# wangjie212/ManiSDP-matlab

Measured on AMD Instinct MI355X. Metric: tCG Hess-vec prods/sec (n,p), G81 MaxCut, higher is better.
Workload: dtype f64; 1 GPU; Gset G81 MaxCut, ManiSDP_onlyunitdiag RTR call, n=20000, p=32; n=20000, p=32, nnz_C=92644, TR_maxiter=40, TR_maxinner=100, parallelism=rows1

## Files before the change

include/manisdp_hip.h:

```cpp
#ifndef MANISDP_HIP_H
#define MANISDP_HIP_H

#include <stdint.h>

#ifdef __cplusplus
extern "C" {
#endif

#define MSDP_OK              0
#define MSDP_EINVAL         -1
#define MSDP_EHIP           -2
#define MSDP_ENOMEM         -3
#define MSDP_ESTATE         -4
#define MSDP_ECOMM          -5
#define MSDP_EUNSUPPORTED   -6

typedef struct msdp_handle_s* msdp_handle;

#define MSDP_KIND_ONLYUNITDIAG 1
#define MSDP_KIND_UNITDIAG     2
#define MSDP_KIND_UNITTRACE    3
#define MSDP_KIND_GENERIC      4
#define MSDP_KIND_MULTIBLOCK   5
#define MSDP_KIND_DUAL_UNITDIAG 6
// ... 137 lines not shown
int msdp_local_rows(msdp_handle h, int64_t* row0, int64_t* row1);


int msdp_al_primal(msdp_handle h, double* obj, double* Ax);
int msdp_al_dual(msdp_handle h, const double* y, double* z);
int msdp_escape_eigs_dual(msdp_handle h, int32_t k, double tol, int32_t maxit,
                          double* lam_min, double* V, double* lam_max, int32_t* iters);
int msdp_get_dual_slack(msdp_handle h, double* S);
int msdp_get_dual_slack_block(msdp_handle h, int64_t row0, int64_t nb, double* S);
int msdp_block_eigs(msdp_handle h, int32_t nb, const int64_t* row0, const int64_t* nblk, int32_t k, int32_t method, double* w, double* V);
#define MSDP_BLOCK_EIGS_LARGE_MAXN 1024
int msdp_block_eigs_large(msdp_handle h, int32_t nb, const int64_t* row0, const int64_t* nblk, int32_t k, double* w, double* V);
int msdp_block_eigs_large_info(msdp_handle h, int32_t* launches, int32_t* workgroups);
#define MSDP_BLOCK_RESHAPE_MAXP 64
int msdp_block_reshape(msdp_handle h, int32_t nb, const int64_t* row0, const int64_t* nblk, const int32_t* p_in,
                       const double* w, const double* V, int32_t k, double theta, int32_t strict, int32_t delta,
                       double alpha, int32_t min_facsize, int32_t mode,
                       int32_t* p_out, int32_t* r_out, int32_t* nne_out, double* U);

int msdp_set_option(msdp_handle h, const char* name, int32_t value);

int msdp_tcg_path(msdp_handle h, int32_t* path);
int msdp_debug_persist_form(msdp_handle h, int32_t* form);


int msdp_bench_hessvec(msdp_handle h, int32_t reps, double* avg_ms,
                       double* algo_bytes, double* algo_flops);
int msdp_bench_kernel(msdp_handle h, int32_t which, int32_t reps, double* avg_ms);
int msdp_bench_tcg_trip(msdp_handle h, int32_t reps, double* avg_ms);

const char* msdp_last_error(void);
const char* msdp_version(void);

#ifdef __cplusplus
}
#endif
#endif
```

manisdp-matlab_amd/_lib.py:

```python
from __future__ import annotations

import ctypes as C
import os

import numpy as np

_HERE = os.path.dirname(os.path.abspath(__file__))
LIB_PATH = os.path.join(_HERE, "lib", "libmanisdp_hip.so")

KIND_ONLYUNITDIAG, KIND_UNITDIAG, KIND_UNITTRACE, KIND_GENERIC, KIND_MULTIBLOCK, KIND_DUAL_UNITDIAG, KIND_DUAL = 1, 2, 3, 4, 5, 6, 7
KIND_DUAL_MULTIBLOCK = 8


class RtrOpts(C.Structure):
    _fields_ = [("maxiter", C.c_int32), ("maxinner", C.c_int32), ("mininner", C.c_int32),
                ("reserved0", C.c_int32), ("tolgradnorm", C.c_double), ("kappa", C.c_double),
                ("theta", C.c_double), ("rho_prime", C.c_double), ("rho_regularization", C.c_double),
                ("Delta_bar", C.c_double), ("Delta0", C.c_double)]


class RtrStats(C.Structure):
    _fields_ = [("cost", C.c_double), ("gradnorm", C.c_double), ("Delta", C.c_double),
                ("seconds", C.c_double), ("iters", C.c_int32), ("hessvecs", C.c_int32),
                ("accepted", C.c_int32), ("rejected", C.c_int32), ("cost_evals", C.c_int32),
# ... 73 lines not shown
    "msdp_comm_init_local": (C.c_int, [C.c_void_p, C.c_int32, C.c_int32, C.c_int32]),
    "msdp_comm_init_ipc": (C.c_int, [C.c_void_p, C.c_int32, C.c_int32, C.c_char_p]),
    "msdp_get_point_all": (C.c_int, [C.c_void_p, _dp]),
    "msdp_get_z_all": (C.c_int, [C.c_void_p, _dp]),
    "msdp_factor_gram": (C.c_int, [C.c_void_p, _dp]),
    "msdp_factor_rotate": (C.c_int, [C.c_void_p, C.c_int32, _dp]),
    "msdp_factor_append": (C.c_int, [C.c_void_p, C.c_int32, _dp, C.c_double, C.c_int32]),
    "msdp_create_dual_unitdiag": (C.c_int, [C.c_int64, C.c_int64, _i64p, _i64p, _dp, _dp, _dp, _dp, C.c_int32, _i64p, _i64p, _dp,
                                            _dp, C.c_int32, C.POINTER(C.c_void_p)]),
    "msdp_create_dual": (C.c_int, [C.c_int64, C.c_int64, _i64p, _i64p, _dp, _dp, _dp, _dp, C.c_int32, _i64p, _i64p, _dp,
                                   _dp, C.c_int32, C.POINTER(C.c_void_p)]),
    "msdp_create_dual_multiblock": (C.c_int, [C.c_int32, _i64p, C.c_int32, C.c_int64, _i64p, _i64p, _dp, _dp, _dp, _dp, C.c_int32,
                                              _i64p, _i64p, _dp, _dp, C.c_int32, C.POINTER(C.c_void_p)]),
    "msdp_dual_info": (C.c_int, [C.c_void_p, _P(C.c_int32)]),
    "msdp_dual_set_penalty": (C.c_int, [C.c_void_p, C.c_double, _dp]),
    "msdp_dual_outer_step": (C.c_int, [C.c_void_p, _dp, _dp, _dp]),
    "msdp_dual_get_y": (C.c_int, [C.c_void_p, _dp]),
    "msdp_comm_unique_id": (C.c_int, [C.c_void_p]),
    "msdp_comm_init": (C.c_int, [C.c_void_p, C.c_int32, C.c_int32, C.c_void_p]),
    "msdp_local_rows": (C.c_int, [C.c_void_p, _i64p, _i64p]),
    "msdp_debug_shard": (C.c_int, [C.c_void_p, C.c_int32, C.c_int32]),
    "msdp_tcg_path": (C.c_int, [C.c_void_p, _P(C.c_int32)]),
    "msdp_debug_persist_form": (C.c_int, [C.c_void_p, _P(C.c_int32)]),
    "msdp_point_snapshot": (C.c_int, [C.c_void_p]),
    "msdp_point_restore": (C.c_int, [C.c_void_p]),
    "msdp_al_primal": (C.c_int, [C.c_void_p, _dp, _dp]),
    "msdp_al_dual": (C.c_int, [C.c_void_p, _dp, _dp]),
    "msdp_escape_eigs_dual": (C.c_int, [C.c_void_p, C.c_int32, C.c_double, C.c_int32, _dp, _dp, _dp, _P(C.c_int32)]),
    "msdp_bench_hessvec": (C.c_int, [C.c_void_p, C.c_int32, _dp, _dp, _dp]),
    "msdp_bench_tcg_trip": (C.c_int, [C.c_void_p, C.c_int32, _dp]),
    "msdp_bench_kernel": (C.c_int, [C.c_void_p, C.c_int32, C.c_int32, _dp]),
    "msdp_last_error": (C.c_char_p, []),
    "msdp_version": (C.c_char_p, []),
}

_lib = None


def load():
    global _lib
    if _lib is not None:
        return _lib
    if not os.path.exists(LIB_PATH):
        raise MsdpError(f"{LIB_PATH} not found: run `python -c 'import __graft_entry__ as g; g.build()'` "
                        "(or `make -C manisdp-matlab_amd/csrc`). There is no CPU fallback.")
    lib = C.CDLL(LIB_PATH)
# ... 1 lines not shown
        fn = getattr(lib, name)
        fn.restype = res
        fn.argtypes = args
    _lib = lib
    import atexit
    atexit.register(lambda: lib.msdp_release_cache())
    return lib


def release_cache():
    _check(load().msdp_release_cache())


def pool_stats():
    a, b, c = C.c_int64(), C.c_int64(), C.c_int64()
    _check(load().msdp_debug_pool_stats(C.byref(a), C.byref(b), C.byref(c)))
    return a.value, b.value, c.value


def mem_info():
    a, b = C.c_int64(), C.c_int64()
    _check(load().msdp_debug_mem_info(C.byref(a), C.byref(b)))
    return a.value, b.value


def _check(rc):
    if rc != 0:
        err = MsdpError(f"libmanisdp_hip error {rc}: {load().msdp_last_error().decode()}")
        err.code = rc
        raise err


def _dptr(a):
    return a.ctypes.data_as(_dp)


def set_device(dev):
    _check(load().msdp_set_device(int(dev)))


def device_count():
    n = C.c_int32()
    _check(load().msdp_device_count(C.byref(n)))
    return n.value


# ... 502 lines not shown
```

manisdp-matlab_amd/csrc/msdp_api.hip:

```cpp
#include "msdp_common.h"
#include <algorithm>
#include <cmath>
#include <cstdarg>
#include <cstdio>
#include <cstdlib>
#include <cstring>

static thread_local char g_err[1024] = "";
void msdp_set_error(const char* fmt, ...) {
    va_list ap;
    va_start(ap, fmt);
    vsnprintf(g_err, sizeof(g_err), fmt, ap);
    va_end(ap);
}
extern "C" const char* msdp_last_error(void) { return g_err; }
extern "C" const char* msdp_version(void) { return "manisdp_hip 0.1.0 (gfx950)"; }

static bool boundary_colmajor(msdp_handle h) { return h->kind == MSDP_KIND_UNITTRACE || h->kind == MSDP_KIND_GENERIC || h->kind == MSDP_KIND_DUAL; }

static void choose_grid(msdp_handle h) {
    Dev& d = h->d;
    int half = d.ld / 2, lpr = 1;
    while (lpr < half && lpr < 64) lpr <<= 1;
    const int rows_per_step = MSDP_WAVES * (64 / lpr);
// ... 95 lines not shown
static int new_handle(int kind, int64_t n, msdp_handle* out) {
    if (!out) { msdp_set_error("out handle pointer is null"); return MSDP_EINVAL; }
    if (n <= 0 || n > 0x7fffffff) { msdp_set_error("matrix order n = %lld out of range", (long long)n); return MSDP_EINVAL; }
    int ndev = 0;
    if (hipGetDeviceCount(&ndev) != hipSuccess || ndev == 0) {
        msdp_set_error("no HIP device visible: libmanisdp_hip has no CPU fallback");
        return MSDP_EHIP;
    }
    msdp_handle h = new msdp_handle_s();
    h->kind = kind;
    h->d.n = (int)n;
    h->d.n_loc = (int)n;
    h->d.row0 = 0;
    h->d.manifold = (kind == MSDP_KIND_UNITTRACE) ? MANI_SPHERE : (kind == MSDP_KIND_GENERIC ? MANI_EUCLID : MANI_OBLIQUE);
    {
        auto on = [](const char* name) { const char* e = getenv(name); return e && atoi(e) != 0; };
        if (on("MSDP_NO_PERSIST")) h->tune.persist = 0;
        if (on("MSDP_NO_FUSED_RTR")) h->tune.fused_rtr = 0;
        if (on("MSDP_NO_PERSIST_PIPE")) h->tune.persist_pipe = 0;
        if (on("MSDP_NO_GRAPH")) h->tune.graph = 0;
        if (on("MSDP_TIMING")) h->tune.timing = 1;
        if (on("MSDP_ESC_DEBUG")) h->tune.esc_debug = 1;
        h->d.persist_ep = h->tune.persist_ep;
        if (const char* e = getenv("MSDP_AFFINE_ROUTE")) h->tune.affine_route = !strcmp(e, "gram") ? 2 : (!strcmp(e, "sddmm") ? 1 : 0);
    }
    hipError_t e = hipSuccess;
    if (!msdp_host_kit_take(h)) {
        e = hipStreamCreateWithFlags(&h->stream, hipStreamNonBlocking);
        if (e == hipSuccess) e = hipHostMalloc((void**)&h->h_ctl, sizeof(Ctl), hipHostMallocDefault);
        if (e == hipSuccess) e = hipHostMalloc((void**)&h->h_frame, 2 * sizeof(Frame), hipHostMallocDefault);
        if (e == hipSuccess) e = hipHostMalloc((void**)&h->h_flags, 64, hipHostMallocDefault);
        if (e == hipSuccess) e = hipHostMalloc((void**)&h->h_status, 64, hipHostMallocMapped);
    }
    if (e == hipSuccess) e = hipEventCreate(&h->ev0);
    if (e == hipSuccess) e = hipEventCreate(&h->ev1);
    if (e == hipSuccess) e = hipEventCreateWithFlags(&h->ev_flag[0], hipEventDisableTiming);
    if (e == hipSuccess) e = hipEventCreateWithFlags(&h->ev_flag[1], hipEventDisableTiming);
    if (e == hipSuccess) {
        *h->h_status = 0;
        void* dp = nullptr;
        e = hipHostGetDevicePointer(&dp, (void*)h->h_status, 0);
        h->d.status = (unsigned long long*)dp;
    }
    if (e != hipSuccess) {
        msdp_set_error("stream/event/pinned setup failed: %s", hipGetErrorString(e));
        delete h;
// ... 653 lines not shown
    if (!name) { msdp_set_error("set_option: null name"); return MSDP_EINVAL; }
    Tuning& t = h->tune;
    if (!strcmp(name, "persist")) t.persist = value != 0;
    else if (!strcmp(name, "fused_rtr")) t.fused_rtr = value != 0;
    else if (!strcmp(name, "graph")) { t.graph = value != 0; h->chunk_len = 0; }
    else if (!strcmp(name, "affine_route")) { if (value < 0 || value > 2) { msdp_set_error("affine_route: 0 auto, 1 sddmm, 2 gram"); return MSDP_EINVAL; } t.affine_route = value; h->chunk_len = 0; h->state_valid = false; }
    else if (!strcmp(name, "timing")) t.timing = value != 0;
    else if (!strcmp(name, "esc_debug")) t.esc_debug = value != 0;
    else if (!strcmp(name, "escape_deflate")) t.escape_deflate = value != 0;
    else if (!strcmp(name, "escape_warm")) t.escape_warm = value != 0;
    else if (!strcmp(name, "escape_start_y")) t.escape_start_y = value != 0;
    else if (!strcmp(name, "xpersist")) t.xpersist = value != 0;
    else if (!strcmp(name, "persist_refresh")) t.persist_refresh = value > 0 ? value : 0;
    else if (!strcmp(name, "xtail")) t.xtail = value ? 1 : 0;
    else if (!strcmp(name, "xr_twolevel")) t.xr_twolevel = value ? 1 : 0;
    else if (!strcmp(name, "window")) { t.window = value < 0 ? 0 : (value > 3 ? 3 : value); h->chunk_len = 0; }
    else if (!strcmp(name, "window_lds")) { t.window_lds = value < 16 ? 16 : (value > 144 ? 144 : value); h->chunk_len = 0; msdp_window_release(h); }
    else if (!strcmp(name, "persist_early")) t.persist_early = value > 0 ? value : 0;
    else if (!strcmp(name, "persist_pipe")) t.persist_pipe = value > 0 ? 1 : 0;
    else if (!strcmp(name, "pipe_refresh")) t.pipe_refresh = value > 0 ? (value < 2 ? 2 : value) : 0;
    else if (!strcmp(name, "pipe_local")) t.pipe_local = value > 0 ? 1 : 0;
    else if (!strcmp(name, "persist_goff")) t.persist_goff = value ? 1 : 0;
    else if (!strcmp(name, "persist_ep")) { t.persist_ep = value ? 1 : 0; h->d.persist_ep = t.persist_ep; h->persist_sig_fn = nullptr; }
    else if (!strcmp(name, "persist_slots")) { t.persist_slots = (value == 3 || value == 4) ? value : 0; h->d.persist_slots = t.persist_slots; }
    else if (!strcmp(name, "psync_backoff")) t.psync_backoff = value > 0 ? value : 0;
    else if (!strcmp(name, "psync8_backoff")) t.psync8_backoff = value > 0 ? (value > 255 ? 255 : value) : 0;
    else if (!strcmp(name, "affine_overlap")) { t.affine_overlap = value != 0; h->chunk_len = 0; }
    else if (!strcmp(name, "trip1")) { t.trip1 = value < 0 ? 0 : (value > 2 ? 2 : value); h->chunk_len = 0; }
    else if (!strcmp(name, "dense_sk")) t.dense_sk = value < 0 ? 0 : value;
    else if (!strcmp(name, "sweep_k")) { t.sweep_k = value < 1 ? 1 : value; choose_grid(h); h->chunk_len = 0; }
    else if (!strcmp(name, "sweep")) { t.sweep = value < 0 ? 0 : (value > 3 ? 3 : value); choose_grid(h); h->chunk_len = 0; }
    else if (!strcmp(name, "trip2")) { t.trip2 = value < 0 ? 0 : (value > 2 ? 2 : value); h->chunk_len = 0; }
    else if (!strcmp(name, "escape_method")) { if (value < 0 || value > 2) { msdp_set_error("escape_method: 0 auto, 1 lanczos, 2 block"); return MSDP_EINVAL; } t.escape_method = value; }
    else if (!strcmp(name, "be_width")) { if (value != 0 && value != 32 && value != 64 && value != 128) { msdp_set_error("be_width: 0, 32, 64 or 128"); return MSDP_EINVAL; } t.be_width = value; }
    else if (!strcmp(name, "be_degree")) t.be_degree = value > 0 ? value : 0;
    else if (!strcmp(name, "be_grid")) t.be_grid = value > 0 ? (value > MSDP_MAX_GRID ? MSDP_MAX_GRID : value) : 0;
    else if (!strcmp(name, "be_lpr")) { if (value != 0 && value != 8 && value != 16 && value != 32 && value != 64) { msdp_set_error("be_lpr: 0, 8, 16, 32 or 64"); return MSDP_EINVAL; } t.be_lpr = value; }
    else if (!strcmp(name, "lanczos_onesync")) t.lanczos_onesync = value != 0;
    else if (!strcmp(name, "lanczos_qglobal")) t.lanczos_qglobal = value != 0;
    else if (!strcmp(name, "block_skip")) t.block_skip = value != 0;
    else if (!strcmp(name, "halo_exchange")) { t.halo_exchange = value != 0; h->state_valid = false; }
    else if (!strcmp(name, "dense_pack")) { t.dense_pack = value != 0; h->chunk_len = 0; }
    else if (!strcmp(name, "affine_fuse")) { t.affine_fuse = value != 0; h->chunk_len = 0; h->state_valid = false; }
    else if (!strcmp(name, "affine_side")) { t.affine_side = value != 0; h->chunk_len = 0; }
    else if (!strcmp(name, "affine_broute")) { t.affine_broute = value != 0; h->chunk_len = 0; }
    else if (!strcmp(name, "dense_sym")) { t.dense_sym = value < 0 ? 0 : (value > 2 ? 2 : value); h->chunk_len = 0; return dense_rereserve(h); }
// ... 269 lines not shown
```

manisdp-matlab_amd/csrc/msdp_common.h:

```cpp
#pragma once
#include <hip/hip_runtime.h>
#include <stdint.h>
#include <string>
#include <vector>
#include "../../include/manisdp_hip.h"

#define MSDP_BLOCK 1024
#define MSDP_WAVES (MSDP_BLOCK / 64)
#define MSDP_MAX_GRID 512
#define MSDP_NPART 12

void msdp_set_error(const char* fmt, ...);

hipError_t msdp_memcpy(void* dst, const void* src, size_t bytes, hipMemcpyKind kind);
hipError_t msdp_memcpy_async(void* dst, const void* src, size_t bytes, hipMemcpyKind kind, hipStream_t s);
hipError_t msdp_memcpy2d(void* dst, size_t dpitch, const void* src, size_t spitch, size_t width, size_t height, hipMemcpyKind kind);
hipError_t msdp_memcpy2d_async(void* dst, size_t dpitch, const void* src, size_t spitch, size_t width, size_t height, hipMemcpyKind kind, hipStream_t s);
void msdp_xfer_release();

#define HIPCHK(expr)                                                              \
    do {                                                                          \
        hipError_t _e = (expr);                                                   \
        if (_e != hipSuccess) {                                                   \
            msdp_set_error("%s failed: %s (%s:%d)", #expr, hipGetErrorString(_e), \
// ... 76 lines not shown
    double* eS[2];
    double* AyU;
    double* Sdual;
    int64_t m;
    const int64_t* at_jc; const int64_t* at_ir; const double* at_pr;
    const int64_t* a_rp;  const int* a_ci;  const double* a_v;
    const double* b; double* yv; double* Axb[2]; double* w;
    double* Pm;
    unsigned long long* status;
    const unsigned char* rowfree;
    const int* blk_lo; const int* blk_hi;
    unsigned long long* trace;
    int xr_gid0, xr_gtot;
    double* xr_rows[4];
    int xr_cap, xr_me, xr_halo;
    const int* xr_ellc; const int* xr_colind; const int* xr_pq; const int* xr_pidx;
    const unsigned long long* xr_paddr;
    int xr_pipe;
    int xr2_on, xr2_n, xr2_me, xr_sys, xr2_skip;
    unsigned long long* xr2_blk;
    unsigned long long* const* xr2_peers;
    int persist_slots;
    int persist_ep;
};

struct Tuning {
    int persist = 1;
    int fused_rtr = 1;
    int graph = 1;
    int affine_route = 0;
    int timing = 0;
    int esc_debug = 0;
    int escape_deflate = 1;
    int escape_start_y = 0;
    int halo_exchange = 0;
    int block_skip = 1;
    int lanczos_qglobal = 0;
    int lanczos_onesync = 1;
    int dense_pack = 1;
    int affine_fuse = 1;
    int affine_side = 1;
    int affine_broute = 1;
    int dense_sym = 1;
    int dense_sym_min = 8192;
    int dense_sym_rt = 0;
    int dense_sym_db = 0;
    int dense_sym_len = 0;
    int dense_sym_res = 0;
    int escape_warm = 1;
    int xpersist = 1;
    int xtail = 1;
    int psync8_backoff = 16;
    int psync_backoff = 19;
    int window = 1;
    int window_lds = 144;
    int persist_refresh = 32;
    int persist_slots = 0;
    int persist_ep = 1;
    int persist_goff = 1;
    int pipe_local = 1;
    int xr_twolevel = 0;
    int pipe_refresh = 16;
    int persist_pipe = 1;
    int persist_early = 0;
    int affine_overlap = 0;
    int dense_sk = 0;
    int sweep_k = 2;
    int sweep = 1;
    int trip1 = 1;
    int trip2 = 1;
    int escape_method = 0;
    int be_width = 0;
    int be_degree = 0;
    int be_grid = 0;
    int be_lpr = 0;
    int grid = 0;
    int blk_groups = 0;
    int fail_block = 0;
    int fail_xr = 0;
    int fail_persist = 0;
};
// ... 249 lines not shown
```

manisdp-matlab_amd/csrc/msdp_persist.hip:

```cpp
#include "msdp_device.h"
#include <math.h>
#include <cstdlib>

#include "msdp_psync.h"

size_t msdp_psync_bytes() { return 2 * PSYNC_REGION * sizeof(double); }

__global__ void k_psync_reset(unsigned long long* slots, int* err) {
    const int tot = (int)PSYNC_CNT_OFF;
    for (int i = blockIdx.x * blockDim.x + threadIdx.x; i < tot; i += gridDim.x * blockDim.x) { slots[i] = PSYNC_SENT; slots[PSYNC_REGION + i] = PSYNC_SENT; }
    if (blockIdx.x == 0 && threadIdx.x < 64) { slots[PSYNC_CNT_OFF + threadIdx.x] = 0ULL; slots[PSYNC_REGION + PSYNC_CNT_OFF + threadIdx.x] = 0ULL; }
    if (blockIdx.x == 0 && threadIdx.x == 0) *err = 0;
}

#define MSDP_TRACE_J0 16
#define MSDP_TRACE_NJ 32
#define TSTAMP(ph) do { if (TRACE && threadIdx.x == 0 && j >= MSDP_TRACE_J0 && j < MSDP_TRACE_J0 + MSDP_TRACE_NJ) \
        d.trace[((size_t)bx * MSDP_TRACE_NJ + (j - MSDP_TRACE_J0)) * 8 + (ph)] = __builtin_readcyclecounter(); } while (0)
template <int LPR, int EW, int R, bool FUSE, bool TRACE, bool XR, bool EARLYP, bool XR2 = false, int EP = 1>
__device__ __forceinline__ void tcg_persist_body(const Dev& d, unsigned long long* slots, int* err, const int bx) {
    static_assert(EP == 1 || (EW == 0 && !XR), "entry-parallel lanes: CSR rows of one rank");
    extern __shared__ double lds[];
    __shared__ double sh[3 * PWAVES];
    __shared__ double shb[8];
// ... 728 lines not shown
        if (pl.ew == 8) return k_tcg_persist_obl<16, 8, 5, false>;
        if (pl.ew == 0) return k_tcg_persist_obl<16, 0, 5, false>;
    }
    if (!fuse && pl.lpr == 32 && pl.r == 5) {
        if (pl.ew == 5) return k_tcg_persist_obl<32, 5, 5, false>;
        if (pl.ew == 8) return k_tcg_persist_obl<32, 8, 5, false>;
        if (pl.ew == 0) return k_tcg_persist_obl<32, 0, 5, false>;
    }
#define PKF(L, E) if (fuse && pl.lpr == L && pl.ew == E && pl.r == L / 4) return k_tcg_persist_obl<L, E, L / 4, true>;
    PKF(8, 5) PKF(8, 8) PKF(16, 5) PKF(16, 8) PKF(8, 0) PKF(16, 0)
    if (fuse) return nullptr;
    PK(8, 5) PK(8, 8) PK(16, 5) PK(16, 8) PK(32, 5) PK(32, 8) PK(8, 0) PK(16, 0) PK(32, 0)
#undef PK
#undef PKF
    return nullptr;
}

static int persist_mode(msdp_handle h) { return h->tune.persist_early ? 1 : (h->tune.persist_pipe ? 2 : 0); }
static bool persist_is_pipe(msdp_handle h, const PersistPlan& pl, bool fuse) { return !h->tune.persist_early && h->tune.persist_pipe && persist_kernel_pipe(pl, fuse) != nullptr; }
static bool persist_is_early(msdp_handle h, const PersistPlan& pl, bool fuse) { return !persist_is_pipe(h, pl, fuse) && h->tune.persist_early && persist_kernel_early(pl, fuse) != nullptr; }
static size_t early_lds(const PersistPlan& pl);
static size_t pipe_lds(const PersistPlan& pl) { const size_t rows = (size_t)pl.r * plan_rstep(pl); return (size_t)pl.ew * rows * sizeof(int) + (size_t)2 * pl.r * PB * sizeof(double2); }

static int persist_grid(const Dev& d) {
    static int cus = -1;
    if (cus < 0) {
        int dev = 0, v = 0;
        if (hipGetDevice(&dev) == hipSuccess &&
            hipDeviceGetAttribute(&v, hipDeviceAttributeMultiprocessorCount, dev) == hipSuccess) cus = v;
        else cus = 0;
        (void)hipGetLastError();
    }
    int g = 256;
    if (g > cus) g = (cus / 8) * 8;
    PersistPlan pl;
    if (g >= 8 && persist_plan(d, g, pl)) {
        const int cap = (pl.ew == 0 ? 1 : pl.r) * plan_rstep(pl);
        int gmin = (((d.n_loc + cap - 1) / cap + 7) / 8) * 8;
        if (gmin < 8) gmin = 8;
        if (gmin < g) g = gmin;
    }
    return g;
}

int msdp_persist_eligible(msdp_handle h) {
    const Dev& d = h->d;
    if (!h->tune.persist || h->persist_failed || h->use_comm || h->nranks != 1 || d.costkind != COST_SPARSE || d.manifold != MANI_OBLIQUE) return 0;
    if (!h->psync_slots) return 0;
    const int G = persist_grid(d);
    if (G < 8) return 0;
    PersistPlan pl;
    if (!persist_plan(d, G, pl)) return 0;
    persist_fn fn = persist_kernel(pl, false, persist_mode(h));
    if (!fn) return 0;
    if (persist_is_early(h, pl, false)) pl.lds += early_lds(pl);
    if (persist_is_pipe(h, pl, false)) pl.lds += pipe_lds(pl);
    if (pl.ew > 0 && d.ellW != pl.ew) return 0;
    if (h->persist_sig_lpr == pl.lpr && h->persist_sig_ew == pl.ew && h->persist_sig_r == pl.r && h->persist_sig_G == G && h->persist_sig_fn == (const void*)fn)
        return h->persist_sig_ok;
    int ok = 0;
    int dev = 0, cus = 0, per_cu = 0;
    if (hipGetDevice(&dev) == hipSuccess &&
// ... 283 lines not shown
```

manisdp-matlab_amd/csrc/msdp_pipe.h:

```cpp
#pragma once
#include <type_traits>
#include "msdp_psync.h"

template <class F>
__device__ __forceinline__ bool psync8(unsigned long long* slots, unsigned gen, int G, double (&v)[8], double* sh8, double* shb8, int* err,
                                       int bid, int backoff, unsigned long long* tr, F on_ready) {
    const int lane = threadIdx.x & 63, w = threadIdx.x >> 6;
    {
        const bool h8 = (lane & 8) != 0;
        double a[4], b[2], x;
#pragma unroll
        for (int k = 0; k < 4; ++k) a[k] = msdp_swap_add<32>(v[k], v[4 + k]);
#pragma unroll
        for (int k = 0; k < 2; ++k) b[k] = msdp_swap_add<16>(a[k], a[2 + k]);
        x = (h8 ? b[1] : b[0]) + msdp_dpp<0x128>(h8 ? b[0] : b[1]);
        x += msdp_dpp<MSDP_DPP_XOR1>(x); x += msdp_dpp<MSDP_DPP_XOR2>(x); x += msdp_dpp<MSDP_DPP_HALF_MIRROR>(x);
        if ((lane & 7) == 0) sh8[(lane >> 3) * PWAVES + w] = x;
    }
    if (tr && threadIdx.x == 0) tr[4] = __builtin_readcyclecounter();
    asm volatile("s_waitcnt vmcnt(0)" ::: "memory");
    __syncthreads();
    if (tr && threadIdx.x == 0) tr[2] = __builtin_readcyclecounter();
    {
        unsigned long long* gbase = slots + (size_t)(gen % PSYNC_GEN) * PSYNC_REP * PSYNC_NV * MSDP_MAX_GRID;
// ... 284 lines not shown
    double bad = 0.0;
#pragma unroll
    for (int i = 0; i < 8; ++i) { v[i] = msdp_readlane(shb8[i], 0); bad += msdp_readlane(shb8[8 + i], 0); }
    return bad == 0.0;
}

#ifndef MSDP_PIPE_LINES
#define MSDP_PIPE_LINES 1
#endif
#if MSDP_PIPE_LINES
#define PSYNC8(slots, gen, G, v, sh8, shb8, err, bid, backoff, tr, f) psync8_lines(slots, gen, G, v, sh8, shp, shb8, err, bid, backoff, tr, f)
#else
#define PSYNC8(slots, gen, G, v, sh8, shb8, err, bid, backoff, tr, f) psync8(slots, gen, G, v, sh8, shb8, err, bid, backoff, tr, f)
#endif
template <int LPR, int EW, int R, bool TRACE, bool FUSE, int XRM = 0, int EP = 1>
__device__ __forceinline__ void tcg_pipe_body(const Dev& d, unsigned long long* slots, int* err, const int bx) {
    constexpr bool XR = XRM != 0, XTWO = XRM == 2;
    constexpr bool CSR = EW == 0;
    static_assert(!XR || (!FUSE && !TRACE), "cross-rank instances: per-iteration launches");
    static_assert(R <= 5, "pipelined trip: every vector in registers");
    static_assert(CSR ? (EP == 64 / LPR && !XR && !TRACE) : EP == 1, "CSR rows: one row per wave, one rank");
    static_assert(PSYNC_NV == 8 && PSYNC_REP * PSYNC_NV == 64, "psync8 posts one slot per lane of wave 0");
    constexpr bool BOFF = !(EW == 8 && LPR == 16), ROWB_INV = !XTWO, UMASK = !(FUSE && LPR == 16);
    extern __shared__ double lds[];
    __shared__ double sh8[8 * PWAVES];
    __shared__ double shp[8 * PWAVES];
    __shared__ double shb8[16];
    constexpr int RPW = 64 / (LPR * EP);
    constexpr int RSTEP = PWAVES * RPW;
    constexpr int ROWS = R * RSTEP;
    double2* Ys = reinterpret_cast<double2*>(lds);
    double2* Gs = Ys + R * PB;
    double* eGs = reinterpret_cast<double*>(Gs + R * PB);
    double* vs = eGs + ROWS;
    int* cs = reinterpret_cast<int*>(vs + EW * ROWS);
    int* ls = cs + EW * ROWS;
    double2* HQs = reinterpret_cast<double2*>(ls + EW * ROWS);
    unsigned long long* pds = reinterpret_cast<unsigned long long*>(HQs + 2 * R * PB);
    double2* YPs = HQs + 2 * R * PB;
    double2* GPs = YPs + R * PB;
    double* EGPs = reinterpret_cast<double*>(GPs + R * PB);

    const Ctl* c = d.ctl;
    const bool lead = bx == 0 && threadIdx.x == 0;
    const int k_tr = c->k;
    if (c->done) {
// ... 25 lines not shown
    const int sub = lane & (LPR - 1), rsub = lane / (LPR * EP);
    const int epi = (lane / LPR) & (EP - 1);
    const bool colok_g = 2 * sub < d.ld;
    const bool colok = colok_g && epi == 0;
    int cur = c->cur;
    const bool bench = c->bench_mode != 0;
    double Delta = c->Delta;
    const double kappa = c->kappa, theta = c->theta;
    const int mininner = c->mininner, maxinner = c->maxinner;
    double gg = c->gg;
    double fx = c->fx;
    int k_it = c->k;
    const double Delta_bar = c->Delta_bar, rho_prime = c->rho_prime, rho_reg_opt = c->rho_reg, tolgradnorm = c->tolgradnorm;
    const int maxiter = c->maxiter;
    int n_acc = c->accepted, n_rej = c->rejected, n_hv = c->hessvecs, n_ce = c->cost_evals;
    const double* __restrict__ Yl = cur ? d.Y[1] : d.Y[0];
    const double* __restrict__ gl = cur ? d.Gr[1] : d.Gr[0];
    const double* __restrict__ eGl = cur ? d.eG[1] : d.eG[0];
    const int slot0 = wave * RPW + rsub;
#define SLOT(r) ((r) * RSTEP + slot0)
#define ROW(r) (lo + SLOT(r))
#define ROK(r) (ROW(r) < hi)
#define OK(r) (ROK(r) && colok)
    const unsigned rowb0 = ((unsigned)(lo + slot0) * (unsigned)d.ld + 2u * (unsigned)sub) * 8u;
#define ROWB(r) (ROWB_INV ? (rowb0 + (unsigned)((r) * RSTEP) * (unsigned)d.ld * 8u) : (((unsigned)ROW(r) * gld + 2 * sub) * 8u))
    const int refresh = c->pipe_refresh;
    const int backoff = (c->psync_backoff & 0xff00ffff) | ((((c->psync_backoff >> 16) & 0xff) ? ((c->psync_backoff >> 16) & 0xff) : (c->psync8_backoff & 0xff)) << 16);
    const double2 zz = make_double2(0.0, 0.0);
    const unsigned gld = (unsigned)d.ld;
    constexpr bool LOC = !CSR && R * EW <= 15;
    constexpr bool MULTI = LOC && !(FUSE && LPR >= 16);
    double2 eta[R], rr[R], md[R], hmd[R], cmd[R], ctr[R];
#pragma unroll
    for (int r = 0; r < R; ++r) {
        const bool rok = ROK(r);
        const int rc = rok ? ROW(r) : lo;
        const int64_t o = (int64_t)rc * d.ld + (colok ? 2 * sub : 0);
        double2 y = ld2(Yl + o), g = ld2(gl + o);
        if (!OK(r)) { y = zz; g = zz; }
        Ys[r * PB + threadIdx.x] = y; Gs[r * PB + threadIdx.x] = g;
        eta[r] = zz; rr[r] = g; md[r] = g; hmd[r] = zz; cmd[r] = zz; ctr[r] = zz;
    }
#pragma unroll 1
    for (int r = 0; r < (CSR ? 0 : R); ++r) {
        const bool rok = ROK(r);
        const int rc = rok ? ROW(r) : lo;
// ... 147 lines not shown
    int j = 0, stop = 5;
    const int k_it0 = c->k;
#define FSTAMP(ph) do { if (TRACE && FUSE && threadIdx.x == 0 && k_it - k_it0 < MSDP_TRACE_NJ) \
        d.trace[((size_t)bx * MSDP_TRACE_NJ + (k_it - k_it0)) * 8 + (ph)] = __builtin_readcyclecounter(); } while (0)
    bool first = true, direct = false, failed = false;
    unsigned xq = 0;
    bool have_x = false;
#define MSDP_TRACE_KSEL 7
#define FTRIP_ON (TRACE && FUSE && k_it - k_it0 == MSDP_TRACE_KSEL && j < MSDP_TRACE_NJ)
#define FTRIP_PTR (d.trace + (size_t)GS * MSDP_TRACE_NJ * 8 + ((size_t)bx * MSDP_TRACE_NJ + j) * 8)
#define PTSTAMP(ph) do { if (!FUSE) { TSTAMP(ph); } else if (FTRIP_ON && threadIdx.x == 0) FTRIP_PTR[ph] = __builtin_readcyclecounter(); } while (0)
  auto trips = [&](auto nlc) {
    constexpr int NL = decltype(nlc)::value;
    constexpr int NG = EW - NL;
#ifndef MSDP_PIPE_VARIANT
#define MSDP_PIPE_VARIANT 0
#endif
    constexpr bool PREF = !CSR && R * NG <= ((FUSE && MSDP_PIPE_VARIANT == 0) ? 9 : 15);
    constexpr bool SPLIT = (MSDP_PIPE_VARIANT == 2 && FUSE) ? true : !PREF;
    double2 X[R][NG > 0 ? NG : 1];
    for (;;) {
        PTSTAMP(0);
#define PIPE_ISSUE(rs, base, w0) do { \
            _Pragma("unroll") for (int r = 0; r < R; ++r) \
            _Pragma("unroll") for (int w = 0; w < NG; ++w) { \
                if ((w0) + w < EW) { \
                    const unsigned coff = (unsigned)cs[((w0) + w) * ROWS + SLOT(r)]; \
                    X[r][w] = ld2_cp<XTWO ? 17 : MSDP_CPOL_SC1>((rs), (base) + (BOFF ? coff + gcol8 : (coff * gld + gcol) * 8u)); } } } while (0)
#define PIPE_FOLDX(r, acc, w0) do { \
            _Pragma("unroll") for (int w = 0; w < NG; ++w) { \
                if ((w0) + w < EW) { \
                    const double vv = vs[((w0) + w) * ROWS + SLOT(r)]; \
                    (acc).x = fma(vv, X[r][w].x, (acc).x); (acc).y = fma(vv, X[r][w].y, (acc).y); } } } while (0)
#define PIPE_FOLDL(r, acc, src) do { \
            _Pragma("unroll") for (int w = 0; w < NL; ++w) { \
                const double vv = vs[w * ROWS + SLOT(r)]; \
                const double2 xx = (src)[(ls[w * ROWS + SLOT(r)] & 0xffffff) + sub]; \
                (acc).x = fma(vv, xx.x, (acc).x); (acc).y = fma(vv, xx.y, (acc).y); } } while (0)
#define PIPE_GATHER_ALL(rs, base, dst) do { \
            if (CSR) { _Pragma("unroll") for (int r = 0; r < R; ++r) (dst)[r] = csr_gather(r, (rs), (base)); break; } \
            _Pragma("unroll") for (int r = 0; r < R; ++r) (dst)[r] = zz; \
            _Pragma("unroll") for (int w0 = 0; w0 < EW; w0 += (NG > 0 ? NG : 1)) { \
                PIPE_ISSUE(rs, base, w0); \
                _Pragma("unroll") for (int r = 0; r < R; ++r) PIPE_FOLDX(r, (dst)[r], w0); } \
            if (!colok) { _Pragma("unroll") for (int r = 0; r < R; ++r) (dst)[r] = zz; } } while (0)
        double v[8] = {0.0, 0.0, 0.0, 0.0, 0.0, 0.0, 0.0, 0.0};
        auto pre_sums = [&]() {
            if (!SPLIT) return;
#pragma unroll
            for (int r = 0; r < R; ++r) {
                const double2 g = Gs[r * PB + threadIdx.x], mdr = md[r], e0 = eta[r], rv = rr[r];
                const double2 rg = make_double2(rv.x - g.x, rv.y - g.y);
                v[3] += mdr.x * g.x + mdr.y * g.y;
                v[5] += mdr.x * rg.x + mdr.y * rg.y;
                v[6] += rv.x * rv.x + rv.y * rv.y;
                v[7] += (e0.x * g.x + e0.y * g.y) + 0.5 * (e0.x * rg.x + e0.y * rg.y);
            }
        };
        if (first) {
            pre_sums();
            PIPE_GATHER_ALL(rs_g, g_base, cmd);
#pragma unroll
            for (int r = 0; r < R; ++r) ctr[r] = cmd[r];
        } else {
            if (direct) {
                PIPE_GATHER_ALL(rs_md, 3u * half_bytes, ctr);
                PIPE_GATHER_ALL(rs_md, 2u * half_bytes, cmd);
            }
            if (!CSR && !have_x) PIPE_ISSUE(rs_md, (xq ^ 1u) * half_bytes, NL);
            pre_sums();
            auto products = [&](auto masked) {
#pragma unroll
                for (int r = 0; r < R; ++r) {
                    double2 a = zz;
                    if (CSR) a = csr_gather(r, rs_md, (xq ^ 1u) * half_bytes);
                    else { PIPE_FOLDL(r, a, HQs + (xq ^ 1u) * R * PB); PIPE_FOLDX(r, a, NL); }
                    if (decltype(masked)::value && !colok) a = zz;
                    ctr[r].x = fma(-alpha, a.x, ctr[r].x); ctr[r].y = fma(-alpha, a.y, ctr[r].y);
                    cmd[r].x = fma(beta, cmd[r].x, ctr[r].x); cmd[r].y = fma(beta, cmd[r].y, ctr[r].y);
                }
            };
            if (UMASK) { if (!CSR && idle_lanes) products(std::true_type()); else products(std::false_type()); } else products(std::true_type());
        }
        have_x = false;
        const bool pub = !first && refresh > 0 && ((j + 1) % refresh) == 0;
#pragma unroll
        for (int r = 0; r < R; ++r) {
            const double2 acc = cmd[r];
            const double2 y = Ys[r * PB + threadIdx.x], mdr = md[r], rv = rr[r];
            const double dot = msdp_group_sum_all<LPR>(acc.x * y.x + acc.y * y.y);
            const double eg = eGs[SLOT(r)];
            double2 hq = make_double2(acc.x - y.x * dot - mdr.x * eg, acc.y - y.y * dot - mdr.y * eg);
            if (!UMASK && !OK(r)) hq = zz;
            hmd[r] = hq;
            if (MULTI) HQs[xq * R * PB + r * PB + threadIdx.x] = hq;
            if (OK(r)) st2_sc1(rs_md, xq * half_bytes + ROWB(r), hq);
            xr_push(r, xq, hq);
            if (pub) {
                const double dn = msdp_group_sum_all<LPR>(rv.x * y.x + rv.y * y.y);
                if (OK(r)) {
                    st2_sc1(rs_md, 2u * half_bytes + ROWB(r), mdr);
                    st2_sc1(rs_md, 3u * half_bytes + ROWB(r), make_double2(rv.x - y.x * dn, rv.y - y.y * dn));
                }
                xr_push(r, 2u, mdr);
                xr_push(r, 3u, make_double2(rv.x - y.x * dn, rv.y - y.y * dn));
            }
            if (!SPLIT) {
                const double2 g = Gs[r * PB + threadIdx.x], e0 = eta[r];
                const double2 rg = make_double2(rv.x - g.x, rv.y - g.y);
                v[0] += mdr.x * hq.x + mdr.y * hq.y;
                v[1] += rv.x * hq.x + rv.y * hq.y;
                v[2] += hq.x * hq.x + hq.y * hq.y;
                v[3] += mdr.x * g.x + mdr.y * g.y;
                v[4] += e0.x * hq.x + e0.y * hq.y;
                v[5] += mdr.x * rg.x + mdr.y * rg.y;
                v[6] += rv.x * rv.x + rv.y * rv.y;
                v[7] += (e0.x * g.x + e0.y * g.y) + 0.5 * (e0.x * rg.x + e0.y * rg.y);
            }
        }
        if (SPLIT) {
#pragma unroll
            for (int r = 0; r < R; ++r) {
                const double2 hq = hmd[r], mdr = md[r], e0 = eta[r], rv = rr[r];
                v[0] += mdr.x * hq.x + mdr.y * hq.y;
                v[1] += rv.x * hq.x + rv.y * hq.y;
                v[2] += hq.x * hq.x + hq.y * hq.y;
                v[4] += e0.x * hq.x + e0.y * hq.y;
            }
        }
        PTSTAMP(1);
        if (TRACE && FUSE && j == 0) { FSTAMP(1); }
        auto next_gather = [&]() { if (PREF && !pub) { PIPE_ISSUE(rs_md, xq * half_bytes, NL); have_x = true; } };
        if (XTWO) {
            if (!psync2_8(d.xr2_blk, shpeer, d.xr2_n, d.xr2_me, xri, gen++, GS + d.xr2_skip, v, sh8, shb8, err, bid, backoff, next_gather)) { failed = true; break; }
        } else
        if (!PSYNC8(slots, gen++, GS, v, sh8, shb8, err, bid, backoff,
                    (TRACE && !FUSE && j >= MSDP_TRACE_J0 && j < MSDP_TRACE_J0 + MSDP_TRACE_NJ) ? d.trace + ((size_t)bx * MSDP_TRACE_NJ + (j - MSDP_TRACE_J0)) * 8 :
                    (FTRIP_ON ? FTRIP_PTR : nullptr),
                    next_gather)) { failed = true; break; }
        PTSTAMP(5);
        const double d_Hd = v[0];
        z_r = v[6];
        model_value = v[7];
        alpha = z_r / d_Hd;
        const double e_Pe_new = e_Pe + 2.0 * alpha * e_Pd + alpha * alpha * d_Pd;
        if (!bench && (d_Hd <= 0.0 || e_Pe_new >= Delta * Delta)) {
            const double tau = (-e_Pd + sqrt(e_Pd * e_Pd + d_Pd * (Delta * Delta - e_Pe))) / d_Pd;
#pragma unroll
            for (int r = 0; r < R; ++r) {
                eta[r].x -= tau * md[r].x; eta[r].y -= tau * md[r].y;
                rr[r].x -= tau * hmd[r].x; rr[r].y -= tau * hmd[r].y;
            }
            stop = (d_Hd <= 0.0) ? 1 : 2;
            ++j;
            break;
        }
        const double new_model = model_value - alpha * v[3] - 0.5 * alpha * (v[4] + v[5]) + 0.5 * alpha * alpha * d_Hd;
        const double r_r = fmax(z_r - 2.0 * alpha * v[1] + alpha * alpha * v[2], 0.0);
        e_Pe = e_Pe_new;
        if (!bench && new_model >= model_value) { stop = 6; ++j; break; }
#pragma unroll
        for (int r = 0; r < R; ++r) {
            eta[r].x -= alpha * md[r].x; eta[r].y -= alpha * md[r].y;
            rr[r].x -= alpha * hmd[r].x; rr[r].y -= alpha * hmd[r].y;
        }
        model_value = new_model;
        ++j;
        const double norm_r = sqrt(r_r);
        const double nr0t = (theta == 1.0) ? norm_r0 : pow(norm_r0, theta);
        if (!bench && j >= mininner && norm_r <= norm_r0 * fmin(nr0t, kappa)) {
            stop = (kappa < nr0t) ? 3 : 4;
            break;
        }
        if (j >= maxinner) break;
        beta = r_r / z_r;
        e_Pd = beta * (e_Pd + alpha * d_Pd);
        d_Pd = r_r + beta * beta * d_Pd;
        z_r = r_r;
#pragma unroll
        for (int r = 0; r < R; ++r) {
            const double2 y = Ys[r * PB + threadIdx.x];
            const double2 vv = make_double2(rr[r].x + beta * md[r].x, rr[r].y + beta * md[r].y);
            const double dot = msdp_group_sum_all<LPR>(vv.x * y.x + vv.y * y.y);
            md[r] = make_double2(vv.x - y.x * dot, vv.y - y.y * dot);
        }
        direct = pub;
        first = false;
        xq ^= 1u;
        { --j; PTSTAMP(6); ++j; }
    }
#undef PIPE_ISSUE
#undef PIPE_FOLDX
#undef PIPE_FOLDL
#undef PIPE_GATHER_ALL
#undef PTSTAMP
#undef FTRIP_ON
#undef FTRIP_PTR
  };
  if (XR && !XTWO && d.xr2_skip && bid == 0) return;
  if (XR) {
#pragma unroll
    for (int r = 0; r < R; ++r) {
        if (OK(r)) st2_sc1(rs_md, 2u * half_bytes + ROWB(r), md[r]);
// ... 27 lines not shown
    if (TRACE && FUSE && threadIdx.x == 0 && k_it - k_it0 < MSDP_TRACE_NJ)
        d.trace[((size_t)bx * MSDP_TRACE_NJ + (k_it - k_it0)) * 8 + 2] = (__builtin_readcyclecounter() & 0x00ffffffffffffffULL) | ((unsigned long long)(j & 0xff) << 56);
    if (!FUSE) {
#pragma unroll
        for (int r = 0; r < R; ++r) {
            if (OK(r)) {
                const int64_t o = (int64_t)ROW(r) * d.ld + 2 * sub;
                const double2 g = Gs[r * PB + threadIdx.x];
                st2(d.eta[0] + o, eta[r]);
                st2(d.Heta[0] + o, make_double2(rr[r].x - g.x, rr[r].y - g.y));
            }
        }
        if (lead) {
            frame_store(&d.F[0], z_r, d_Pd, e_Pd, e_Pe, model_value, norm_r0, alpha, beta, 0, j, stop, 0, 0, 0);
            d.ctl->tcg_running = 0;
            msdp_publish(d, k_tr, j, 0);
        }
        return;
    }
    double tv[8] = {0.0, 0.0, 0.0, 0.0, 0.0, 0.0, 0.0, 0.0};
    const unsigned yx_base = 4u * half_bytes, gx_base = (5u + (unsigned)(cur ^ 1)) * half_bytes;
#pragma unroll
    for (int r = 0; r < R; ++r) {
        const double2 y = Ys[r * PB + threadIdx.x], g = Gs[r * PB + threadIdx.x];
        const double2 e0 = eta[r];
        const double2 he = make_double2(rr[r].x - g.x, rr[r].y - g.y);
        tv[2] += e0.x * (g.x + 0.5 * he.x) + e0.y * (g.y + 0.5 * he.y);
        const double2 x = make_double2(y.x + e0.x, y.y + e0.y);
        double nn = sqrt(msdp_group_sum_all<LPR>(x.x * x.x + x.y * x.y));
        if (!(nn > 0.0)) nn = 1.0;
        const double2 ypr = OK(r) ? make_double2(x.x / nn, x.y / nn) : zz;
        YPs[r * PB + threadIdx.x] = ypr;
        if (OK(r)) st2_sc1(rs_md, yx_base + ROWB(r), ypr);
    }
    FSTAMP(3);
    if (!pbar8_lines(slots, gen++, GS, shb8, err, bid, backoff)) return;
    FSTAMP(4);
    auto prop_finish = [&](int r, double2 acc) {
        if (!colok) acc = zz;
        const double2 ypr = YPs[r * PB + threadIdx.x];
        const double dot = msdp_group_sum_all<LPR>(acc.x * ypr.x + acc.y * ypr.y);
        const double2 gpr = OK(r) ? make_double2(acc.x - ypr.x * dot, acc.y - ypr.y * dot) : zz;
        GPs[r * PB + threadIdx.x] = gpr;
        tv[1] += gpr.x * gpr.x + gpr.y * gpr.y;
        if (sub == 0 && epi == 0) {
            EGPs[SLOT(r)] = ROK(r) ? dot : 0.0;
            if (ROK(r)) tv[0] += 0.5 * dot;
        }
        if (OK(r)) st2_sc1(rs_md, gx_base + ROWB(r), gpr);
    };
    if (CSR) {
#pragma unroll
        for (int r = 0; r < R; ++r) prop_finish(r, csr_gather(r, rs_md, yx_base));
    } else if (R * EW <= 16) {
        double2 XG[R][EW > 0 ? EW : 1];
#pragma unroll
        for (int r = 0; r < R; ++r)
#pragma unroll
            for (int w = 0; w < EW; ++w) XG[r][w] = ld2_sc1(rs_md, yx_base + (BOFF ? (unsigned)cs[w * ROWS + SLOT(r)] + gcol8 : ((unsigned)cs[w * ROWS + SLOT(r)] * gld + gcol) * 8u));
#pragma unroll
        for (int r = 0; r < R; ++r) {
            double2 acc = zz;
#pragma unroll
            for (int w = 0; w < EW; ++w) { const double vv = vs[w * ROWS + SLOT(r)]; acc.x = fma(vv, XG[r][w].x, acc.x); acc.y = fma(vv, XG[r][w].y, acc.y); }
            prop_finish(r, acc);
        }
    } else {
#pragma unroll 1
        for (int r = 0; r < R; ++r) {
            double2 xw[EW > 0 ? EW : 1];
#pragma unroll
            for (int w = 0; w < EW; ++w) xw[w] = ld2_sc1(rs_md, yx_base + (BOFF ? (unsigned)cs[w * ROWS + SLOT(r)] + gcol8 : ((unsigned)cs[w * ROWS + SLOT(r)] * gld + gcol) * 8u));
            double2 acc = zz;
#pragma unroll
            for (int w = 0; w < EW; ++w) { const double vv = vs[w * ROWS + SLOT(r)]; acc.x = fma(vv, xw[w].x, acc.x); acc.y = fma(vv, xw[w].y, acc.y); }
            prop_finish(r, acc);
        }
    }
    FSTAMP(5);
    if (!PSYNC8(slots, gen++, GS, tv, sh8, shb8, err, bid, backoff, nullptr, []() {})) return;
    FSTAMP(6);
    {
        const double fp = tv[0], ggp = tv[1], prd = tv[2];
        double rhonum = fx - fp;
        double rhoden = -prd;
        const double rreg = fmax(1.0, fabs(fx)) * 2.220446049250313e-16 * rho_reg_opt;
        rhonum += rreg;
        rhoden += rreg;
        const bool model_decreased = rhoden >= 0.0;
        const double rho = rhonum / rhoden;
        if (rho < 0.25 || !model_decreased || isnan(rho)) Delta = Delta / 4.0;
        else if (rho > 0.75 && (stop == 1 || stop == 2)) Delta = fmin(2.0 * Delta, Delta_bar);
// ... 23 lines not shown
    {
        double* Yo = cur ? d.Y[1] : d.Y[0];
        double* Go = cur ? d.Gr[1] : d.Gr[0];
        double* eo = cur ? d.eG[1] : d.eG[0];
#pragma unroll
        for (int r = 0; r < R; ++r) {
            if (OK(r)) {
                const int64_t o = (int64_t)ROW(r) * d.ld + 2 * sub;
                st2(Yo + o, Ys[r * PB + threadIdx.x]);
                st2(Go + o, Gs[r * PB + threadIdx.x]);
            }
            if (sub == 0 && ROK(r)) eo[ROW(r)] = eGs[SLOT(r)];
        }
    }
    if (lead) {
        Ctl* cw = d.ctl;
        cw->fx = fx; cw->gg = gg; cw->norm_grad = sqrt(gg); cw->Delta = Delta;
        cw->k = k_it; cw->cur = cur;
        cw->done = 1;
        cw->tcg_running = 0;
        frame_store(&d.F[0], 0.0, 0.0, 0.0, 0.0, 0.0, 0.0, 0.0, 0.0, 0, 0, stop, 0, 0, 0);
    }
#undef FSTAMP
#undef SLOT
#undef ROW
#undef ROK
#undef OK
#undef ROWB
}

template <int LPR, int EW, int R, bool TRACE = false, bool FUSE = false, int XRM = 0, int EP = 1>
__global__ __launch_bounds__(PB) void k_tcg_pipe_obl(Dev d, unsigned long long* slots, int* err) {
    tcg_pipe_body<LPR, EW, R, TRACE, FUSE, XRM, EP>(d, slots, err, (int)blockIdx.x);
}
```

Before: 198,600 Hess-vec/s.

## Balance persistent grid row slots and skip empty trailing row slots per wave

Adds a grid-size search that picks a persistent grid size (same slot count per block) minimizing the maximum number of row slots any wave pair must process. In the pipelined tCG kernel, for EW=5 configurations, each wave computes how many of its R row slots are actually in range and skips gather, fold and vector-update work for an empty last slot. The aim is to reduce the imbalance in which some waves do a full extra row slot of padded work while others idle at barriers. It adds a wave-uniform branch in the hot loop and may change the grid size, which could affect occupancy or sync cost.

```diff
diff --git a/include/manisdp_hip.h b/include/manisdp_hip.h
--- a/include/manisdp_hip.h
+++ b/include/manisdp_hip.h
@@ -183,6 +183,7 @@
 
 int msdp_tcg_path(msdp_handle h, int32_t* path);
 int msdp_debug_persist_form(msdp_handle h, int32_t* form);
+int msdp_persist_balanced_grid(int n_loc, int gmin, int gmax, int rstep, int r);
 
 
 int msdp_bench_hessvec(msdp_handle h, int32_t reps, double* avg_ms,
diff --git a/manisdp-matlab_amd/_lib.py b/manisdp-matlab_amd/_lib.py
--- a/manisdp-matlab_amd/_lib.py
+++ b/manisdp-matlab_amd/_lib.py
@@ -119,6 +119,7 @@
     "msdp_debug_shard": (C.c_int, [C.c_void_p, C.c_int32, C.c_int32]),
     "msdp_tcg_path": (C.c_int, [C.c_void_p, _P(C.c_int32)]),
     "msdp_debug_persist_form": (C.c_int, [C.c_void_p, _P(C.c_int32)]),
+    "msdp_persist_balanced_grid": (C.c_int, [C.c_int, C.c_int, C.c_int, C.c_int, C.c_int]),
     "msdp_point_snapshot": (C.c_int, [C.c_void_p]),
     "msdp_point_restore": (C.c_int, [C.c_void_p]),
     "msdp_al_primal": (C.c_int, [C.c_void_p, _dp, _dp]),
@@ -166,6 +167,10 @@
     a, b = C.c_int64(), C.c_int64()
     _check(load().msdp_debug_mem_info(C.byref(a), C.byref(b)))
     return a.value, b.value
+
+
+def persist_balanced_grid(n_loc, gmin, gmax, rstep, r):
+    return int(load().msdp_persist_balanced_grid(int(n_loc), int(gmin), int(gmax), int(rstep), int(r)))
 
 
 def _check(rc):
diff --git a/manisdp-matlab_amd/csrc/msdp_api.hip b/manisdp-matlab_amd/csrc/msdp_api.hip
--- a/manisdp-matlab_amd/csrc/msdp_api.hip
+++ b/manisdp-matlab_amd/csrc/msdp_api.hip
@@ -141,6 +141,7 @@
         if (on("MSDP_TIMING")) h->tune.timing = 1;
         if (on("MSDP_ESC_DEBUG")) h->tune.esc_debug = 1;
         h->d.persist_ep = h->tune.persist_ep;
+        h->d.persist_balance = h->tune.persist_balance;
         if (const char* e = getenv("MSDP_AFFINE_ROUTE")) h->tune.affine_route = !strcmp(e, "gram") ? 2 : (!strcmp(e, "sddmm") ? 1 : 0);
     }
     hipError_t e = hipSuccess;
@@ -840,6 +841,7 @@
     else if (!strcmp(name, "pipe_local")) t.pipe_local = value > 0 ? 1 : 0;
     else if (!strcmp(name, "persist_goff")) t.persist_goff = value ? 1 : 0;
     else if (!strcmp(name, "persist_ep")) { t.persist_ep = value ? 1 : 0; h->d.persist_ep = t.persist_ep; h->persist_sig_fn = nullptr; }
+    else if (!strcmp(name, "persist_balance")) { t.persist_balance = value ? 1 : 0; h->d.persist_balance = t.persist_balance; h->persist_sig_fn = nullptr; h->fused_sig_fn = nullptr; }
     else if (!strcmp(name, "persist_slots")) { t.persist_slots = (value == 3 || value == 4) ? value : 0; h->d.persist_slots = t.persist_slots; }
     else if (!strcmp(name, "psync_backoff")) t.psync_backoff = value > 0 ? value : 0;
     else if (!strcmp(name, "psync8_backoff")) t.psync8_backoff = value > 0 ? (value > 255 ? 255 : value) : 0;
diff --git a/manisdp-matlab_amd/csrc/msdp_common.h b/manisdp-matlab_amd/csrc/msdp_common.h
--- a/manisdp-matlab_amd/csrc/msdp_common.h
+++ b/manisdp-matlab_amd/csrc/msdp_common.h
@@ -122,6 +122,7 @@
     unsigned long long* const* xr2_peers;
     int persist_slots;
     int persist_ep;
+    int persist_balance;
 };
 
 struct Tuning {
@@ -157,6 +158,7 @@
     int persist_refresh = 32;
     int persist_slots = 0;
     int persist_ep = 1;
+    int persist_balance = 1;
     int persist_goff = 1;
     int pipe_local = 1;
     int xr_twolevel = 0;
diff --git a/manisdp-matlab_amd/csrc/msdp_persist.hip b/manisdp-matlab_amd/csrc/msdp_persist.hip
--- a/manisdp-matlab_amd/csrc/msdp_persist.hip
+++ b/manisdp-matlab_amd/csrc/msdp_persist.hip
@@ -774,6 +774,30 @@
 static size_t early_lds(const PersistPlan& pl);
 static size_t pipe_lds(const PersistPlan& pl) { const size_t rows = (size_t)pl.r * plan_rstep(pl); return (size_t)pl.ew * rows * sizeof(int) + (size_t)2 * pl.r * PB * sizeof(double2); }
 
+extern "C" int msdp_persist_balanced_grid(int n_loc, int gmin, int gmax, int rstep, int r) {
+    if (n_loc < 1 || gmin < 1 || rstep < PWAVES) return gmin;
+    const int rpw = rstep / PWAVES;
+    auto cost = [&](int rows) {
+        int c = 0;
+        for (int k = 0; k < PWAVES / 2; ++k) {
+            int s = 0;
+            for (int w = k; w < PWAVES; w += PWAVES / 2) { const int left = rows - w * rpw; if (left > 0) s += (left + rstep - 1) / rstep; }
+            if (s > c) c = s;
+        }
+        return c;
+    };
+    const int rows0 = (n_loc + gmin - 1) / gmin, slots0 = (rows0 + rstep - 1) / rstep;
+    if (slots0 != r) return gmin;
+    int best = gmin, cbest = cost(rows0);
+    for (int g = gmin + 8; g <= gmax; g += 8) {
+        const int rows = (n_loc + g - 1) / g;
+        if ((rows + rstep - 1) / rstep != slots0) break;
+        const int cg = cost(rows);
+        if (cg < cbest) { cbest = cg; best = g; }
+    }
+    return best;
+}
+
 static int persist_grid(const Dev& d) {
     static int cus = -1;
     if (cus < 0) {
@@ -790,6 +814,7 @@
         const int cap = (pl.ew == 0 ? 1 : pl.r) * plan_rstep(pl);
         int gmin = (((d.n_loc + cap - 1) / cap + 7) / 8) * 8;
         if (gmin < 8) gmin = 8;
+        if (pl.ew != 0 && pl.lpr == 16 && d.persist_balance != 0 && gmin < g) gmin = msdp_persist_balanced_grid(d.n_loc, gmin, g, plan_rstep(pl), pl.r);
         if (gmin < g) g = gmin;
     }
     return g;
diff --git a/manisdp-matlab_amd/csrc/msdp_pipe.h b/manisdp-matlab_amd/csrc/msdp_pipe.h
--- a/manisdp-matlab_amd/csrc/msdp_pipe.h
+++ b/manisdp-matlab_amd/csrc/msdp_pipe.h
@@ -330,6 +330,7 @@
     static_assert(CSR ? (EP == 64 / LPR && !XR && !TRACE) : EP == 1, "CSR rows: one row per wave, one rank");
     static_assert(PSYNC_NV == 8 && PSYNC_REP * PSYNC_NV == 64, "psync8 posts one slot per lane of wave 0");
     constexpr bool BOFF = !(EW == 8 && LPR == 16), ROWB_INV = !XTWO, UMASK = !(FUSE && LPR == 16);
+    constexpr bool WSKIP = !XR && EW == 5 && ((LPR == 16 && R == 3) || (LPR == 8 && R == 2));
     extern __shared__ double lds[];
     __shared__ double sh8[8 * PWAVES];
     __shared__ double shp[8 * PWAVES];
@@ -401,6 +402,14 @@
 #define ROW(r) (lo + SLOT(r))
 #define ROK(r) (ROW(r) < hi)
 #define OK(r) (ROK(r) && colok)
+    int nrs = R;
+    if (WSKIP && d.persist_balance != 0) {
+        int nmine = 0;
+#pragma unroll
+        for (int r = 0; r < R; ++r) if (lo + r * RSTEP + wave * RPW < hi) nmine = r + 1;
+        nrs = __builtin_amdgcn_readfirstlane(nmine);
+    }
+#define RUN(r) (!WSKIP || (r) < R - 1 || nrs == R)
     const unsigned rowb0 = ((unsigned)(lo + slot0) * (unsigned)d.ld + 2u * (unsigned)sub) * 8u;
 #define ROWB(r) (ROWB_INV ? (rowb0 + (unsigned)((r) * RSTEP) * (unsigned)d.ld * 8u) : (((unsigned)ROW(r) * gld + 2 * sub) * 8u))
     const int refresh = c->pipe_refresh;
@@ -594,7 +603,7 @@
     for (;;) {
         PTSTAMP(0);
 #define PIPE_ISSUE(rs, base, w0) do { \
-            _Pragma("unroll") for (int r = 0; r < R; ++r) \
+            _Pragma("unroll") for (int r = 0; r < R; ++r) if (RUN(r)) \
             _Pragma("unroll") for (int w = 0; w < NG; ++w) { \
                 if ((w0) + w < EW) { \
                     const unsigned coff = (unsigned)cs[((w0) + w) * ROWS + SLOT(r)]; \
@@ -614,13 +623,14 @@
             _Pragma("unroll") for (int r = 0; r < R; ++r) (dst)[r] = zz; \
             _Pragma("unroll") for (int w0 = 0; w0 < EW; w0 += (NG > 0 ? NG : 1)) { \
                 PIPE_ISSUE(rs, base, w0); \
-                _Pragma("unroll") for (int r = 0; r < R; ++r) PIPE_FOLDX(r, (dst)[r], w0); } \
+                _Pragma("unroll") for (int r = 0; r < R; ++r) if (RUN(r)) PIPE_FOLDX(r, (dst)[r], w0); } \
             if (!colok) { _Pragma("unroll") for (int r = 0; r < R; ++r) (dst)[r] = zz; } } while (0)
         double v[8] = {0.0, 0.0, 0.0, 0.0, 0.0, 0.0, 0.0, 0.0};
         auto pre_sums = [&]() {
             if (!SPLIT) return;
 #pragma unroll
             for (int r = 0; r < R; ++r) {
+                if (!RUN(r)) continue;
                 const double2 g = Gs[r * PB + threadIdx.x], mdr = md[r], e0 = eta[r], rv = rr[r];
                 const double2 rg = make_double2(rv.x - g.x, rv.y - g.y);
                 v[3] += mdr.x * g.x + mdr.y * g.y;
@@ -644,6 +654,7 @@
             auto products = [&](auto masked) {
 #pragma unroll
                 for (int r = 0; r < R; ++r) {
+                    if (!RUN(r)) continue;
                     double2 a = zz;
                     if (CSR) a = csr_gather(r, rs_md, (xq ^ 1u) * half_bytes);
                     else { PIPE_FOLDL(r, a, HQs + (xq ^ 1u) * R * PB); PIPE_FOLDX(r, a, NL); }
@@ -658,6 +669,7 @@
         const bool pub = !first && refresh > 0 && ((j + 1) % refresh) == 0;
 #pragma unroll
         for (int r = 0; r < R; ++r) {
+            if (!RUN(r)) continue;
             const double2 acc = cmd[r];
             const double2 y = Ys[r * PB + threadIdx.x], mdr = md[r], rv = rr[r];
             const double dot = msdp_group_sum_all<LPR>(acc.x * y.x + acc.y * y.y);
@@ -693,6 +705,7 @@
         if (SPLIT) {
 #pragma unroll
             for (int r = 0; r < R; ++r) {
+                if (!RUN(r)) continue;
                 const double2 hq = hmd[r], mdr = md[r], e0 = eta[r], rv = rr[r];
                 v[0] += mdr.x * hq.x + mdr.y * hq.y;
                 v[1] += rv.x * hq.x + rv.y * hq.y;
@@ -720,6 +733,7 @@
             const double tau = (-e_Pd + sqrt(e_Pd * e_Pd + d_Pd * (Delta * Delta - e_Pe))) / d_Pd;
 #pragma unroll
             for (int r = 0; r < R; ++r) {
+                if (!RUN(r)) continue;
                 eta[r].x -= tau * md[r].x; eta[r].y -= tau * md[r].y;
                 rr[r].x -= tau * hmd[r].x; rr[r].y -= tau * hmd[r].y;
             }
@@ -733,6 +747,7 @@
         if (!bench && new_model >= model_value) { stop = 6; ++j; break; }
 #pragma unroll
         for (int r = 0; r < R; ++r) {
+            if (!RUN(r)) continue;
             eta[r].x -= alpha * md[r].x; eta[r].y -= alpha * md[r].y;
             rr[r].x -= alpha * hmd[r].x; rr[r].y -= alpha * hmd[r].y;
         }
@@ -751,6 +766,7 @@
         z_r = r_r;
 #pragma unroll
         for (int r = 0; r < R; ++r) {
+            if (!RUN(r)) continue;
             const double2 y = Ys[r * PB + threadIdx.x];
             const double2 vv = make_double2(rr[r].x + beta * md[r].x, rr[r].y + beta * md[r].y);
             const double dot = msdp_group_sum_all<LPR>(vv.x * y.x + vv.y * y.y);
@@ -824,6 +840,7 @@
     const unsigned yx_base = 4u * half_bytes, gx_base = (5u + (unsigned)(cur ^ 1)) * half_bytes;
 #pragma unroll
     for (int r = 0; r < R; ++r) {
+        
         const double2 y = Ys[r * PB + threadIdx.x], g = Gs[r * PB + threadIdx.x];
         const double2 e0 = eta[r];
         const double2 he = make_double2(rr[r].x - g.x, rr[r].y - g.y);
@@ -862,6 +879,7 @@
             for (int w = 0; w < EW; ++w) XG[r][w] = ld2_sc1(rs_md, yx_base + (BOFF ? (unsigned)cs[w * ROWS + SLOT(r)] + gcol8 : ((unsigned)cs[w * ROWS + SLOT(r)] * gld + gcol) * 8u));
 #pragma unroll
         for (int r = 0; r < R; ++r) {
+            
             double2 acc = zz;
 #pragma unroll
             for (int w = 0; w < EW; ++w) { const double vv = vs[w * ROWS + SLOT(r)]; acc.x = fma(vv, XG[r][w].x, acc.x); acc.y = fma(vv, XG[r][w].y, acc.y); }
@@ -870,6 +888,7 @@
     } else {
 #pragma unroll 1
         for (int r = 0; r < R; ++r) {
+            
             double2 xw[EW > 0 ? EW : 1];
 #pragma unroll
             for (int w = 0; w < EW; ++w) xw[w] = ld2_sc1(rs_md, yx_base + (BOFF ? (unsigned)cs[w * ROWS + SLOT(r)] + gcol8 : ((unsigned)cs[w * ROWS + SLOT(r)] * gld + gcol) * 8u));
@@ -939,6 +958,7 @@
         frame_store(&d.F[0], 0.0, 0.0, 0.0, 0.0, 0.0, 0.0, 0.0, 0.0, 0, 0, stop, 0, 0, 0);
     }
 #undef FSTAMP
+#undef RUN
 #undef SLOT
 #undef ROW
 #undef ROK
```

After: 199,700 Hess-vec/s (median of 2 runs). No clear change (+0.5%).
